# toybox-rs/Toybox

Hardware: AMD Instinct MI355X
Metric: env steps/sec (whole node), Breakout 64k-env batch (higher is better)
Workload: dtype f64

## Files before the change

toybox_amd/csrc/breakout.hip:

```cpp

#include "tbx_common.hpp"
#include "raster.hpp"
#include "agent_device.hpp"

#include <cstdlib>
#include <cstring>
#include <vector>

namespace {

constexpr int MAXB = TBX_BRK_MAX_BALLS;
constexpr int MAXK = TBX_BRK_MAX_BRICKS / 64;

struct BrkCustom {
    double x[TBX_BRK_MAX_BRICKS], y[TBX_BRK_MAX_BRICKS], w[TBX_BRK_MAX_BRICKS], h[TBX_BRK_MAX_BRICKS];
    int32_t points[TBX_BRK_MAX_BRICKS], depth[TBX_BRK_MAX_BRICKS], row[TBX_BRK_MAX_BRICKS], col[TBX_BRK_MAX_BRICKS];
    uint32_t color[TBX_BRK_MAX_BRICKS];
    uint8_t destructible[TBX_BRK_MAX_BRICKS];
};

struct BrkDev {
    int n;
    uint64_t* sim_rng;
    int32_t* prev_score;
// ... 1237 lines not shown
    const BrkRenderRec* __restrict__ recs, BrkPalette pal, uint8_t* __restrict__ out, int count, int split, BrkDev d, const BrkCfg* __restrict__ cp,
    ActionSource src, uint32_t flags, BrkRenderRec* __restrict__ recs_next, int step_blocks, unsigned long long* arrive, int release_block, int diag)
{
    if (!OVL) {
        if ((int)blockIdx.x < step_blocks) {
            const int env = (int)blockIdx.x * TBX_BLOCK + (int)threadIdx.x;
            if (env < d.n) brk_step_tpe_body<false, false>(d, *cp, src, flags, recs_next, nullptr, nullptr, env);
            return;
        }
        brk_render_body<C, false, false>(recs, nullptr, pal, out, 0, count, split | (1 << 16), nullptr, nullptr, (int)blockIdx.x - step_blocks);
        return;
    }
    if ((int)blockIdx.x < step_blocks) {
        const int env = (int)blockIdx.x * TBX_BLOCK + (int)threadIdx.x;
        if (OVL_DIAG(diag, 1)) {
            __builtin_amdgcn_fence(__ATOMIC_ACQUIRE, "agent");
            if (env < d.n) brk_step_tpe_body<false, false>(d, *cp, src, flags, recs_next, nullptr, nullptr, env);
            if (!OVL_DIAG(diag, 2)) __threadfence();
        } else {
            if (env < d.n) brk_step_tpe_body<false, true>(d, *cp, src, flags, recs_next, nullptr, nullptr, env);
            __builtin_amdgcn_s_waitcnt(0x0F70);
        }
        __syncthreads();
        if (threadIdx.x == 0) __hip_atomic_fetch_add(arrive, 1ull, __ATOMIC_RELAXED, __HIP_MEMORY_SCOPE_AGENT);
        return;
    }
    if ((int)blockIdx.x == release_block && threadIdx.x == 0) __hip_atomic_fetch_add(arrive + 1, 1ull, __ATOMIC_RELAXED, __HIP_MEMORY_SCOPE_AGENT);
    brk_render_body<C, false, false, true>(recs, nullptr, pal, out, 0, count, split | (1 << 16) | (OVL_DIAG(diag, 4) ? 1 << 17 : 0), nullptr, nullptr, (int)blockIdx.x - step_blocks);
}

template <int C, bool CUSTOM, bool ALT>
__global__ __launch_bounds__(TBX_BLOCK) void brk_render_kernel(const BrkRenderRec* __restrict__ recs, const BrkCustom* __restrict__ custom, BrkPalette pal,
                                                               uint8_t* __restrict__ out, int first_env, int count, int split,
                                                               const BrkRenderRec* __restrict__ recs_alt = nullptr, const uint8_t* __restrict__ pick_alt = nullptr)
{
    brk_render_body<C, CUSTOM, ALT>(recs, custom, pal, out, first_env, count, split, recs_alt, pick_alt, (int)blockIdx.x);
}

template <bool CUSTOM>
__device__ __forceinline__ bool brk_serve_paint(const BrkDev& d, const BrkRenderRec* recs, const BrkPalette& pal, int channels, uint8_t* frame, int lane, uint8_t* lds,
                                                int part, int split)
{
    const BrkRecLanes rec{brk_rec_load_lanes(&recs[0], lane)};
    switch (channels) {
    case 1: brk_paint_units<1, CUSTOM>(rec, d.custom, pal, BrkLaneTables<1>(pal, lane), frame, 0, lane, RowStager<1, TBX_BRK_W, BRK_UNIT_ROWS>{lds}, part, split); break;
    case 3: brk_paint_units<3, CUSTOM>(rec, d.custom, pal, BrkLaneTables<3>(pal, lane), frame, 0, lane, RowStager<3, TBX_BRK_W, BRK_UNIT_ROWS>{lds}, part, split); break;
    default: brk_paint_units<4, CUSTOM>(rec, d.custom, pal, BrkLaneTables<4>(pal, lane), frame, 0, lane, RowStager<4, TBX_BRK_W, BRK_UNIT_ROWS>{lds}, part, split); break;
    }
    return true;
}

template <bool CUSTOM>
__global__ __launch_bounds__(64 * TBX_SERVE_WAVES) void brk_serve_kernel(BrkDev d, BrkCfg c, BrkRenderRec* recs, BrkPalette pal, TbxServeCtl* ctl)
{
    __shared__ __attribute__((aligned(16))) uint8_t lds[TBX_SERVE_WAVES][RowStager<4, TBX_BRK_W, BRK_UNIT_ROWS>::UNIT_BYTES];
    const int lane = threadIdx.x & 63, wave = threadIdx.x >> 6;
    tbx_serve_loop(ctl, lane,
                   [&](const ActionSource& src, uint32_t flags) {
                       brk_step_body<CUSTOM>(d, c, src, flags, 0, lane);
                       __threadfence();
                       if (lane == 0) recs[0] = brk_record_of(d, 0);
                   },
                   [&](int channels, uint8_t* frame, int part, int split) { return brk_serve_paint<CUSTOM>(d, recs, pal, channels, frame, lane, lds[wave], part, split); },
                   d.reward, d.done, d.lives_out, d.score_out, d.err_flag);
}

__global__ __launch_bounds__(64 * TBX_SERVE_WAVES) void brk_serve_tpe_kernel(BrkDev d, const BrkCfg* __restrict__ cp, BrkRenderRec* recs, BrkPalette pal, TbxServeCtl* ctl)
{
    __shared__ __attribute__((aligned(16))) uint8_t lds[TBX_SERVE_WAVES][RowStager<4, TBX_BRK_W, BRK_UNIT_ROWS>::UNIT_BYTES];
    const int lane = threadIdx.x & 63, wave = threadIdx.x >> 6;
    tbx_serve_loop(ctl, lane, [&](const ActionSource& src, uint32_t flags) { if (lane == 0) brk_step_tpe_body<false>(d, *cp, src, flags, recs, nullptr, nullptr, 0); },
                   [&](int channels, uint8_t* frame, int part, int split) { return brk_serve_paint<false>(d, recs, pal, channels, frame, lane, lds[wave], part, split); },
                   d.reward, d.done, d.lives_out, d.score_out, d.err_flag);
}


struct BrkGrayPal {
    uint32_t bg, frame, paddle, ball;
    int32_t rows;
    uint32_t row[TBX_BRK_MAX_ROWS];
    uint64_t boundary[3];
};

struct BrkLineCache { int row; uint32_t dw; };

__device__ __forceinline__ uint32_t brk_gray_line(const BrkRenderRec& rec, const BrkGrayPal& pal, int y, int x0, uint32_t side_dw,
                                                  const uint32_t (&hud)[4], BrkLineCache& bc, bool has_overlay)
{
    uint32_t d;
    if (y < TBX_BRK_WALL_Y0) d = pal.bg * 0x01010101u;
    else if (y < TBX_BRK_WALL_Y0 + 12) d = pal.frame * 0x01010101u;
    else d = side_dw;
    const int by = y - 43;
    if (by >= 0 && by < 4 * pal.rows) {
        const int row = by >> 2;
        if (row != bc.row) {
            bc.row = row;
            uint32_t b = side_dw;
#pragma unroll
            for (int i = 0; i < 4; i++) {
                const int bxp = x0 + i - 12;
                if (bxp >= 0 && bxp < 216) {
                    const int j = (bxp / 12) * pal.rows + row;
                    const uint64_t w = sel4(j >> 6, rec.alive[0], rec.alive[1], rec.alive[2], rec.alive[3]);
                    if ((w >> (j & 63)) & 1ull) b = (b & ~(0xFFu << (8 * i))) | (pal.row[row] << (8 * i));
                }
            }
            bc.dw = b;
        }
        d = bc.dw;
    }
#pragma unroll
    for (int k = 0; k < 1 + MAXB; k++) {
        if (!has_overlay) break;
        const uint32_t rc = k == 0 ? rec.paddle : rec.ball[k - 1];
        const int ry0 = (int)((rc >> 16) & 255u), ry1 = (int)(rc >> 24);
        if (y >= ry0 && y < ry1) {
            const int rx0 = (int)(rc & 255u), rx1 = (int)((rc >> 8) & 255u);
            const uint32_t col = (k == 0 ? pal.paddle : pal.ball) * 0x01010101u;
            uint32_t m = 0;
#pragma unroll
            for (int i = 0; i < 4; i++)
                if (x0 + i >= rx0 && x0 + i < rx1) m |= 0xFFu << (8 * i);
            d = (d & ~m) | (col & m);
        }
    }
    if (y >= 2 && y < 12) {
        const int gr = ((y - 2) >> 1) * 3;
        uint32_t m = 0;
#pragma unroll
        for (int i = 0; i < 4; i++)
            if ((hud[i] >> gr) & 1u) m |= 0xFFu << (8 * i);
        d = (d & ~m) | ((pal.frame * 0x01010101u) & m);
    }
    return d;
}

template <int S>
__global__ __launch_bounds__(TBX_BLOCK) __attribute__((amdgpu_waves_per_eu(5))) void brk_agent_warp_kernel(const BrkRenderRec* __restrict__ recsLive, const BrkRenderRec* __restrict__ recsA,
                                                                   const BrkRenderRec* __restrict__ recsB, const BrkRenderRec* __restrict__ keepA,
                                                                   const BrkRenderRec* __restrict__ keepB, BrkGrayPal pal, AgentWarpArgs a, int n)
{
    constexpr int W = TBX_BRK_W, H = TBX_BRK_H;
    __shared__ __attribute__((aligned(16))) uint8_t lds_all[TBX_WAVES_PER_BLOCK][352];
    __shared__ __attribute__((aligned(16))) uint8_t vals_all[TBX_WAVES_PER_BLOCK][AGENT_MAX_OUT_PX];
    const int lane = threadIdx.x & 63;
    const int wave = threadIdx.x >> 6;
    const int env = wave_uniform(a.first + blockIdx.x * TBX_WAVES_PER_BLOCK + wave);
    if (env >= a.end) return;
    uint8_t* row = lds_all[wave];
    uint8_t* vals = vals_all[wave];
    const ObsSel sel = agent_obs_sel(a, env);
    if (sel.none) {
        for (int i = lane; i < a.oh * a.ow; i += 64) vals[i] = 0;
        observation_commit<S>(vals, a, env, lane, sel.zero);
        return;
    }
    const bool fresh = !sel.two;
    const BrkRenderRec* __restrict__ srcA = sel.keep ? keepA : recsA;
    const BrkRenderRec* __restrict__ srcB = sel.single == 0 ? recsLive : sel.single == 1 ? srcA : sel.keep ? keepB : recsB;
    const BrkRenderRec recA = srcA[env];
    const BrkRenderRec recB = srcB[env];
    const int x0 = lane * 4;
    const bool active = x0 < W;
    const uint32_t half = (uint32_t)(H * W) / 2u;
    const ColTaps c0 = load_col(a.tx, lane, a.ow), c1 = load_col(a.tx, lane + 64, a.ow);
    const bool on0 = lane < a.ow, on1 = lane + 64 < a.ow;
    if (lane < 8) reinterpret_cast<uint32_t*>(row)[80 + lane] = 0u;
    if (lane >= 60 && lane < 64) reinterpret_cast<uint32_t*>(row)[lane] = 0u;
    if (lane < 16) reinterpret_cast<uint32_t*>(row)[64 + lane] = 0u;

    uint32_t side_dw = 0;
#pragma unroll
    for (int i = 0; i < 4; i++) side_dw |= ((x0 + i < 12 || x0 + i >= 228) ? pal.frame : pal.bg) << (8 * i);
    uint32_t hudA[4], hudB[4];
    {
        const int hud_x0[7] = {36, 44, 52, 60, 68, 148, 196};
#pragma unroll
        for (int i = 0; i < 4; i++) {
            uint32_t sel = 7u << 2;
#pragma unroll
            for (int g = 0; g < 7; g++) {
                const int dx = x0 + i - hud_x0[g];
                if (dx >= 0 && dx < 6) sel = ((uint32_t)g << 2) | (uint32_t)(dx >> 1);
            }
            const uint32_t g = sel >> 2;
            const uint32_t ga = g < 7 ? tbx_digit_glyph((recA.hud >> (4 * g)) & 15u) : 0u;
            const uint32_t gb = g < 7 ? tbx_digit_glyph((recB.hud >> (4 * g)) & 15u) : 0u;
            hudA[i] = (ga >> (sel & 3u)) & 0x1249u;
            hudB[i] = (gb >> (sel & 3u)) & 0x1249u;
        }
    }

    BrkLineCache bcA{-1, 0}, bcB{-1, 0};
    uint64_t need[3] = {pal.boundary[0], pal.boundary[1], pal.boundary[2]};
    uint64_t ovA[3] = {0, 0, 0}, ovB[3] = {0, 0, 0}, diff_a[3] = {0, 0, 0};
    {
        brk_overlay_rows(recB, ovB);
        if (!fresh) brk_overlay_rows(recA, ovA);
        uint64_t ov[3];
#pragma unroll
        for (int w = 0; w < 3; w++) { ov[w] = ovA[w] | ovB[w]; need[w] |= ov[w]; diff_a[w] = fresh ? 0ull : ov[w]; }
        if (!fresh) {
            if (recA.alive[0] != recB.alive[0] || recA.alive[1] != recB.alive[1] || recA.alive[2] != recB.alive[2] ||
                recA.alive[3] != recB.alive[3] || recA.n_bricks != recB.n_bricks)
                brk_mark_rows(diff_a, 43, 43 + 4 * pal.rows);
            if (recA.hud != recB.hud) brk_mark_rows(diff_a, 2, 12);
        }
        need[2] |= (ov[2] << 1) | (ov[1] >> 63);
        need[1] |= (ov[1] << 1) | (ov[0] >> 63);
        need[0] |= (ov[0] << 1) | 1ull;
    }
    uint32_t h0 = 0, h1 = 0;
    uint32_t acc[2] = {0, 0};
    int oy = 0, top = H, pos = 0;
    auto run_to = [&](int end) {
        while (top <= end) {
            const uint32_t w = (uint32_t)(top - pos);
            const uint32_t s0 = acc[0] + __umul24(w, h0), s1 = acc[1] + __umul24(w, h1);
            if (on0) vals[oy * a.ow + lane] = (uint8_t)(((uint64_t)(s0 + half) * a.magic) >> 42);
            if (on1) vals[oy * a.ow + lane + 64] = (uint8_t)(((uint64_t)(s1 + half) * a.magic) >> 42);
            acc[0] = 0; acc[1] = 0;
            pos = top; top += H; oy += 1;
        }
        const uint32_t w = (uint32_t)(end - pos);
        acc[0] += __umul24(w, h0); acc[1] += __umul24(w, h1);
        pos = end;
    };
#pragma unroll 1
    for (int wi = 0; wi < 3; wi++) {
        uint64_t nw = sel4(wi, need[0], need[1], need[2], 0ull);
        const uint64_t oa = sel4(wi, ovA[0], ovA[1], ovA[2], 0ull), ob = sel4(wi, ovB[0], ovB[1], ovB[2], 0ull);
        const uint64_t da = sel4(wi, diff_a[0], diff_a[1], diff_a[2], 0ull);
        if (wi == 2) nw &= (1ull << (H - 128)) - 1ull;
#pragma unroll 1
        for (; nw; nw &= nw - 1ull) {
            const int b = (int)__builtin_ctzll(nw), sy = 64 * wi + b;
            run_to(sy * a.oh);
            const uint32_t dB = brk_gray_line(recB, pal, sy, x0, side_dw, hudB, bcB, (ob >> b) & 1ull);
            uint32_t v = dB;
            if ((da >> b) & 1ull) v = bytemax4(brk_gray_line(recA, pal, sy, x0, side_dw, hudA, bcA, (oa >> b) & 1ull), dB);
            if (active) reinterpret_cast<uint32_t*>(row)[lane] = v;
            __builtin_amdgcn_wave_barrier();
            h0 = on0 ? hsum(row, c0) : 0u;
            h1 = on1 ? hsum(row, c1) : 0u;
            __builtin_amdgcn_wave_barrier();
        }
    }
    run_to(H * a.oh);
    observation_commit<S>(vals, a, env, lane, sel.zero);
}


template <bool CUSTOM>
__global__ void brk_pack_kernel(BrkDev d, BrkCfg c, int env, tbx_breakout_state_t* out)
{
    env += blockIdx.x;
    out += blockIdx.x;
    const int lane = threadIdx.x & 63;
    BrkRegs s;
    brk_load(d, env, lane, s);
    if (lane == 0) {
        out->rand[0] = s.rng.s0; out->rand[1] = s.rng.s1;
        out->score = s.score; out->lives = s.lives; out->level = s.level;
        out->is_dead = (s.flags & 1) ? 1 : 0; out->reset = (s.flags & 2) ? 1 : 0;
        out->_pad0[0] = out->_pad0[1] = 0;
        out->paddle_x = s.px; out->paddle_y = s.py; out->paddle_vx = s.pvx; out->paddle_vy = s.pvy;
        out->paddle_width = s.pw; out->paddle_speed = s.pspeed; out->ball_radius = s.radius;
        out->n_balls = s.n_balls; out->n_bricks = s.n_bricks;
        for (int b = 0; b < MAXB; b++) {
            out->ball_x[b] = s.bx[b]; out->ball_y[b] = s.by[b]; out->ball_vx[b] = s.bvx[b]; out->ball_vy[b] = s.bvy[b];
        }
    }
    for (int k = 0; k < MAXK; k++) {
        const int j = lane + 64 * k;
        tbx_brick_t b;
        memset(&b, 0, sizeof b);
        if (j < s.n_bricks) {
            if (CUSTOM) {
                const BrkCustom& t = d.custom[env];
                b.x = t.x[j]; b.y = t.y[j]; b.w = t.w[j]; b.h = t.h[j];
                b.points = t.points[j]; b.depth = t.depth[j]; b.row = t.row[j]; b.col = t.col[j];
                b.color = unpack_color(t.color[j]); b.destructible = t.destructible[j];
            } else {
                int row, col;
                brk_canon(j, c.n_rows, row, col, b.x, b.y);
                b.w = TBX_BRK_BRICK_W; b.h = TBX_BRK_BRICK_H;
                b.points = c.row_scores[row]; b.depth = c.n_rows - 1 - row; b.row = row; b.col = col;
                b.color = unpack_color(c.row_colors[row]); b.destructible = 1;
            }
            b.alive = (s.mybits >> k) & 1u;
        }
        out->bricks[j] = b;
    }
}

template <bool CUSTOM>
__global__ void brk_unpack_kernel(BrkDev d, int env, const tbx_breakout_state_t* in)
{
    env += blockIdx.x;
    in += blockIdx.x;
    const int lane = threadIdx.x & 63;
    BrkRegs s;
    s.rng.s0 = in->rand[0]; s.rng.s1 = in->rand[1];
    s.score = in->score; s.lives = in->lives; s.level = in->level;
    s.flags = (in->is_dead ? 1 : 0) | (in->reset ? 2 : 0);
    s.px = in->paddle_x; s.py = in->paddle_y; s.pvx = in->paddle_vx; s.pvy = in->paddle_vy;
    s.pw = in->paddle_width; s.pspeed = in->paddle_speed; s.radius = in->ball_radius;
    s.n_balls = in->n_balls; s.n_bricks = in->n_bricks;
    for (int b = 0; b < MAXB; b++) {
        const bool v = b < s.n_balls;
        s.bx[b] = v ? in->ball_x[b] : 0.0; s.by[b] = v ? in->ball_y[b] : 0.0;
        s.bvx[b] = v ? in->ball_vx[b] : 0.0; s.bvy[b] = v ? in->ball_vy[b] : 0.0;
    }
    uint32_t bits = 0;
    for (int k = 0; k < MAXK; k++) {
        const int j = lane + 64 * k;
        const tbx_brick_t& b = in->bricks[j];
        if (j < s.n_bricks && b.alive) bits |= 1u << k;
        if (CUSTOM) {
            BrkCustom& t = d.custom[env];
            const bool v = j < s.n_bricks;
            t.x[j] = v ? b.x : 0.0; t.y[j] = v ? b.y : 0.0; t.w[j] = v ? b.w : 0.0; t.h[j] = v ? b.h : 0.0;
            t.points[j] = v ? b.points : 0; t.depth[j] = v ? b.depth : 0; t.row[j] = v ? b.row : 0; t.col[j] = v ? b.col : 0;
            t.color[j] = v ? pack_color(b.color) : 0u; t.destructible[j] = v ? (b.destructible ? 1 : 0) : 0;
        }
    }
    s.mybits = bits;
    brk_store(d, env, lane, s);
}

__global__ __launch_bounds__(TBX_BLOCK) void brk_fill_custom_kernel(BrkDev d, BrkCfg c)
{
// ... 90 lines not shown
        o[0] = c;
        break;
    }
    case TBX_QUERY_BRK_NUM_BRICKS: o[0] = nb; break;
    case TBX_QUERY_BRK_COLUMN: case TBX_QUERY_BRK_ROW: {
        const int key = a.geti(env, 0);
        int m = 0;
        for (int j = 0; j < nb && m < width; j++) {
            int row, col;
            brk_brick_rc<CUSTOM>(d, env, j, rows, row, col);
            if ((query == TBX_QUERY_BRK_COLUMN ? col : row) == key) o[m++] = alive(j);
        }
        for (; m < width; m++) o[m] = -1.0;
        break;
    }
    case TBX_QUERY_BRK_IS_CHANNEL: case TBX_QUERY_BRK_CHANNEL_COUNT: case TBX_QUERY_BRK_FIND_CHANNEL: {
        const int ncols = query == TBX_QUERY_BRK_IS_CHANNEL ? 0 : (rows > 0 ? nb / rows : 0);
        const int want = a.geti(env, 0);
        int count = 0, first = -1, is = 0;
        const int c0 = query == TBX_QUERY_BRK_IS_CHANNEL ? want : 0, c1 = query == TBX_QUERY_BRK_IS_CHANNEL ? want + 1 : ncols;
        for (int cc = c0; cc < c1; cc++) {
            int bricks = 0, live = 0;
            for (int j = 0; j < nb; j++) {
                int row, col;
                brk_brick_rc<CUSTOM>(d, env, j, rows, row, col);
                if (col == cc) { bricks++; live += alive(j); }
            }
            if (bricks > 0 && live == 0) { count++; if (first < 0) first = cc; is = 1; }
        }
        o[0] = query == TBX_QUERY_BRK_IS_CHANNEL ? is : query == TBX_QUERY_BRK_CHANNEL_COUNT ? count : first;
        break;
    }
    case TBX_QUERY_BRK_FIND_BRICK: {
        const int want = a.geti(env, 0);
        int first = -1;
        for (int j = 0; j < nb && first < 0; j++)
            if (((a.getu(env, 1 + (j >> 5)) >> (j & 31)) & 1u) && (want < 0 || alive(j) == (want != 0))) first = j;
        o[0] = first;
        break;
    }
    case TBX_QUERY_BRK_PADDLE:
        for (int i = 0; i < 4; i++) o[i] = d.paddle[(size_t)i * N + env];
        break;
    case TBX_QUERY_BRK_BALLS: {
        const int n = d.n_balls[env];
        o[0] = n;
        for (int f = 0; f < 4; f++)
            for (int b = 0; b < MAXB; b++) o[1 + f * MAXB + b] = b < n ? d.balls[(size_t)(f * MAXB + b) * N + env] : -1.0;
        break;
    }
    default: break;
    }
}

__global__ void brk_scalars_kernel(BrkDev d, int32_t* score, int32_t* lives, int32_t* level)
{
    const int i = blockIdx.x * blockDim.x + threadIdx.x;
    if (i >= d.n) return;
    if (score) score[i] = d.score[i];
    if (lives) lives[i] = d.lives[i];
    if (level) level[i] = d.level[i];
}


struct BrkSlots {
    BrkRenderRec *recsA, *recsB;
    BrkRenderRec *keepA, *keepB;
    template <class F>
    constexpr void arrays(F&& f)
    {
        f(recsA, tbx_rows(sizeof(BrkRenderRec))); f(recsB, tbx_rows(sizeof(BrkRenderRec)));
        f(keepA, tbx_rows(sizeof(BrkRenderRec))); f(keepB, tbx_rows(sizeof(BrkRenderRec)));
    }
};
static_assert(sizeof(BrkSlots) == sizeof(void*) * tbx_array_count<BrkSlots>(), "BrkSlots: the arrays of arrays()");

struct BreakoutOps : GameOps {
    BrkDev d{};
    BrkCfg c{};
    tbx_breakout_config_t cfg{};
    bool custom = false;
    TbxRecordSet<BrkRenderRec> recs;
    BrkCfg* cfg_dev = nullptr;

    static void default_config(tbx_breakout_config_t* k);

    int height() const override { return TBX_BRK_H; }
    int width() const override { return TBX_BRK_W; }
    size_t state_size() const override { return sizeof(tbx_breakout_state_t); }
    size_t config_size() const override { return sizeof(tbx_breakout_config_t); }

    int load_cfg(tbx_engine* e, const tbx_breakout_config_t& k)
    {
        if (k.n_rows < 1 || k.n_rows > TBX_BRK_MAX_ROWS) return e->fail(TBX_E_UNSUPPORTED, "breakout: n_rows must be 1..14");
        if (k.n_starts < 1 || k.n_starts > TBX_BRK_MAX_STARTS) return e->fail(TBX_E_UNSUPPORTED, "breakout: 1..8 ball_start_positions");
        if (k.paddle_discrete_segments < 1 || k.paddle_discrete_segments > TBX_BRK_MAX_SEGMENTS)
            return e->fail(TBX_E_UNSUPPORTED, "breakout: paddle_discrete_segments must be 1..16 (continuous bounce needs device trig)");
        cfg = k;
        c.start_lives = k.start_lives; c.n_rows = k.n_rows; c.ball_speed_row_depth = k.ball_speed_row_depth;
        c.n_starts = k.n_starts; c.segments = k.paddle_discrete_segments;
        for (int i = 0; i < TBX_BRK_MAX_ROWS; i++) { c.row_scores[i] = k.row_scores[i]; c.row_colors[i] = pack_color(k.row_colors[i]); }
        c.speed_slow = k.ball_speed_slow; c.speed_fast = k.ball_speed_fast;
        for (int i = 0; i < TBX_BRK_MAX_STARTS; i++) {
            c.start_x[i] = k.start_x[i]; c.start_y[i] = k.start_y[i];
            c.start_dx[i] = k.start_dir_x[i]; c.start_dy[i] = k.start_dir_y[i];
        }
        for (int i = 0; i < TBX_BRK_MAX_SEGMENTS; i++) { c.pad_dx[i] = k.paddle_dir_x[i]; c.pad_dy[i] = k.paddle_dir_y[i]; }
        c.bg = pack_color(k.bg_color); c.frame = pack_color(k.frame_color);
        c.paddle = pack_color(k.paddle_color); c.ball = pack_color(k.ball_color);
        if (!cfg_dev) TBX_HIP(hipMalloc((void**)&cfg_dev, sizeof(BrkCfg)));
        TBX_HIP(hipMemcpy(cfg_dev, &c, sizeof(BrkCfg), hipMemcpyHostToDevice));
        return TBX_OK;
    }

    int init(tbx_engine* e, const void* cfg_pod, size_t cfg_size) override
    {
        tbx_breakout_config_t k;
        if (cfg_pod) {
            if (cfg_size != sizeof k) return e->fail(TBX_E_INVALID, "breakout: config size mismatch");
            memcpy(&k, cfg_pod, sizeof k);
        } else {
            return e->fail(TBX_E_INVALID, "breakout: a config record is required");
        }
        int rc = load_cfg(e, k);
        if (rc) return rc;
        options_changed(e);
        tbx_bind_engine(d, e);
        TBX_HIP(tbx_alloc_arrays(d, (size_t)e->n));
        TBX_HIP(recs.alloc((size_t)e->n, 3));
        return TBX_OK;
    }

    void destroy(tbx_engine*) override
    {
        tbx_free_arrays(d);
        tbx_free_arrays(slots);
        recs.release();
        hipFree(cfg_dev);
    }

    int get_config(tbx_engine*, void* pod) override { memcpy(pod, &cfg, sizeof cfg); return TBX_OK; }
    int set_config(tbx_engine* e, const void* pod) override
    {
        tbx_breakout_config_t k;
        memcpy(&k, pod, sizeof k);
        return load_cfg(e, k);
    }

    int new_game(tbx_engine* e, const uint8_t* mask_dev, hipStream_t s) override
    {
        tbx_dispatch<0, 1>(custom, [&](auto cu) { hipLaunchKernelGGL(brk_new_game_kernel<decltype(cu)::value != 0>, grid_for(e->n), dim3(TBX_BLOCK), 0, s, d, c, mask_dev); });
        TBX_HIP(hipGetLastError());
        recs.valid = false;
        return TBX_OK;
    }

    int step(tbx_engine* e, const ActionSource& src, uint32_t flags, hipStream_t s) override
    {
        if (!custom && src.single_env < 0 && use_tpe) {
            if (src.acc_reward || src.buf_valid || src.exec_flag || src.frames > 1) {
                if (flags & TBX_STEP_AUTO_RESET) return e->fail(TBX_E_INVALID, "an agent step cannot auto-reset");
                hipLaunchKernelGGL(brk_step_tpe_kernel<true>, dim3((e->n + 127) / 128), dim3(128), 0, s, d, cfg_dev, src, flags, recs.cur, slots.recsA, slots.recsB);
            } else
                TBX_LAUNCH_STEP(e, s, (brk_step_tpe_kernel<false>), dim3((e->n + 127) / 128), dim3(128), d, cfg_dev, src, flags, recs.cur, slots.recsA, slots.recsB);
            TBX_HIP(hipGetLastError());
            recs.valid = true;
// ... 131 lines not shown
            tbx_dispatch<0, 1>(custom, [&](auto cu) {
                tbx_dispatch<0, 1>(pick_alt != nullptr, [&](auto al) {
                    if (C >= 3) BRK_LAUNCH(brk_render_kernel_w5);
                    else BRK_LAUNCH(brk_render_kernel);
                });
            });
#undef BRK_LAUNCH
        };
        constexpr int HEAD_ENVS = 1024;
        if (two_parts) { launch_part(0, HEAD_ENVS); launch_part(HEAD_ENVS, count - HEAD_ENVS); }
        else launch_part(0, count);
    }

    int render(tbx_engine* e, uint8_t* out_dev, int channels, int first_env, int n_envs, hipStream_t s) override
    {
        if (!tbx_dispatch<1, 3, 4>(channels, [&](auto ch) { launch_render<decltype(ch)::value>(out_dev, first_env, n_envs, s); }))
            return e->fail(TBX_E_INVALID, "channels must be 1, 3 or 4");
        TBX_HIP(hipGetLastError());
        return TBX_OK;
    }

    BrkSlots slots{};

    bool agent_fused() const override { return !custom; }
    bool multi_frame_step() const override { return !custom && use_tpe; }
    bool agent_reset_supported() const override { return !custom; }

    int agent_prepare(tbx_engine* e) override
    {
        if (!slots.recsA) TBX_HIP(tbx_alloc_arrays(slots, (size_t)e->n));
        TBX_HIP(tbx_zero_arrays(slots, (size_t)e->n));
        return TBX_OK;
    }

    int agent_snapshot(tbx_engine* e, int slot, const uint8_t* exec_flag, uint8_t* buf_valid, hipStream_t s) override
    {
        hipLaunchKernelGGL(brk_render_prep_kernel, dim3((e->n + 255) / 256), dim3(256), 0, s, d, slot ? slots.recsB : slots.recsA, 0, e->n, exec_flag,
                           buf_valid, slot ? 2 : 1);
        TBX_HIP(hipGetLastError());
        return TBX_OK;
    }

    int render_from(tbx_engine* e, int source, const uint8_t* pick_live, uint8_t* out_dev, int channels, hipStream_t s) override
    {
        const BrkRenderRec* src_recs = source == 1 ? slots.recsA : source == 2 ? slots.recsB : nullptr;
        const BrkRenderRec* alt = (src_recs && pick_live) ? recs.cur : nullptr;
        if (!tbx_dispatch<1, 3, 4>(channels, [&](auto ch) { launch_render<decltype(ch)::value>(out_dev, 0, e->n, s, src_recs, alt, alt ? pick_live : nullptr); }))
            return e->fail(TBX_E_INVALID, "channels must be 1, 3 or 4");
        TBX_HIP(hipGetLastError());
        return TBX_OK;
    }

    int agent_reset_envs(tbx_engine* e, const AgentResetArgs& r, hipStream_t s) override
    {
        if (custom) return e->fail(TBX_E_UNSUPPORTED, "breakout: episodic-life / fire-reset / no-op-reset need the canonical brick wall");
        hipLaunchKernelGGL(brk_agent_reset_kernel, dim3((e->n + 127) / 128), dim3(128), 0, s, d, cfg_dev, r, recs.cur, slots.recsA, slots.recsB, slots.keepA, slots.keepB);
        TBX_HIP(hipGetLastError());
        return TBX_OK;
    }

    static uint32_t host_gray(uint32_t rgba)
    {
        const uint32_t r = rgba & 255u, g = (rgba >> 8) & 255u, b = (rgba >> 16) & 255u;
        return (77u * r + 150u * g + 29u * b + 128u) >> 8;
    }

    int agent_warp(tbx_engine* e, const AgentWarpArgs& a, hipStream_t s) override
    {
        BrkGrayPal pal;
        pal.bg = host_gray(c.bg); pal.frame = host_gray(c.frame); pal.paddle = host_gray(c.paddle); pal.ball = host_gray(c.ball);
        pal.rows = c.n_rows;
        for (int i = 0; i < TBX_BRK_MAX_ROWS; i++) pal.row[i] = host_gray(c.row_colors[i]);
        pal.boundary[0] = pal.boundary[1] = pal.boundary[2] = 0;
        auto mark = [&](int y) { if (y >= 0 && y < TBX_BRK_H) pal.boundary[y >> 6] |= 1ull << (y & 63); };
        mark(0);
        for (int y = 2; y <= 12; y += 2) mark(y);
        mark(TBX_BRK_WALL_Y0); mark(TBX_BRK_WALL_Y0 + 12);
        for (int r = 0; r <= c.n_rows; r++) mark(43 + 4 * r);
        if (!recs.valid) {
            hipLaunchKernelGGL(brk_render_prep_kernel, dim3((e->n + 255) / 256), dim3(256), 0, s, d, recs.cur, 0, e->n);
            TBX_HIP(hipGetLastError());
            recs.valid = true;
        }
        const dim3 grid = grid_for(a.end - a.first), block(TBX_BLOCK);
        tbx_dispatch<0, 1, 2, 3, 4>(tbx_stack_arm(a.obs, a.stack), [&](auto depth) {
            hipLaunchKernelGGL(brk_agent_warp_kernel<decltype(depth)::value>, grid, block, 0, s, recs.cur, slots.recsA, slots.recsB, slots.keepA, slots.keepB, pal, a, e->n);
        });
        TBX_HIP(hipGetLastError());
        return TBX_OK;
    }

    int pack_state(tbx_engine* e, int env, int count, hipStream_t s) override
    {
        auto* out = (tbx_breakout_state_t*)e->staging.p;
        tbx_dispatch<0, 1>(custom, [&](auto cu) { hipLaunchKernelGGL(brk_pack_kernel<decltype(cu)::value != 0>, dim3(count), dim3(64), 0, s, d, c, env, out); });
        TBX_HIP(hipGetLastError());
        return TBX_OK;
    }

    bool is_canonical(const tbx_breakout_state_t& st) const
    {
        if (st.n_bricks != TBX_BRK_COLS * cfg.n_rows) return false;
        for (int j = 0; j < st.n_bricks; j++) {
            const tbx_brick_t& b = st.bricks[j];
            const int col = j / cfg.n_rows, row = j % cfg.n_rows;
            if (b.x != TBX_BRK_LEFT + TBX_BRK_BRICK_W * col || b.y != TBX_BRK_BRICK_Y0 + TBX_BRK_BRICK_H * row ||
                b.w != TBX_BRK_BRICK_W || b.h != TBX_BRK_BRICK_H || b.points != cfg.row_scores[row] ||
                b.depth != cfg.n_rows - 1 - row || b.row != row || b.col != col || !b.destructible ||
                pack_color(b.color) != pack_color(cfg.row_colors[row]))
                return false;
        }
        return true;
    }

    int enable_custom(tbx_engine* e, hipStream_t s)
    {
        if (custom) return TBX_OK;
        TBX_HIP(tbx_alloc_arrays(d, (size_t)e->n, true));
        hipLaunchKernelGGL(brk_fill_custom_kernel, grid_for(e->n), dim3(TBX_BLOCK), 0, s, d, c);
        TBX_HIP(hipGetLastError());
        custom = true;
        return TBX_OK;
    }

    int unpack_state(tbx_engine* e, int env, int count, const void* pod_host, hipStream_t s) override
    {
        const auto* sts = (const tbx_breakout_state_t*)pod_host;
        bool all_canonical = true;
        for (int i = 0; i < count; i++) {
            const auto& st = sts[i];
            if (st.n_balls < 0 || st.n_balls > TBX_BRK_MAX_BALLS)
                return e->fail(TBX_E_UNSUPPORTED, "breakout: the device engine holds at most 4 balls per env");
            if (st.n_bricks < 0 || st.n_bricks > TBX_BRK_MAX_BRICKS)
                return e->fail(TBX_E_UNSUPPORTED, "breakout: the device engine holds at most 256 bricks per env");
            if (!custom && all_canonical && !is_canonical(st)) all_canonical = false;
        }
        if (!custom && !all_canonical) {
            int rc = enable_custom(e, s);
            if (rc) return rc;
        }
        TBX_HIP(hipMemcpyAsync(e->staging.p, pod_host, sizeof(tbx_breakout_state_t) * (size_t)count, hipMemcpyHostToDevice, s));
        auto* in = (const tbx_breakout_state_t*)e->staging.p;
        tbx_dispatch<0, 1>(custom, [&](auto cu) { hipLaunchKernelGGL(brk_unpack_kernel<decltype(cu)::value != 0>, dim3(count), dim3(64), 0, s, d, env, in); });
        TBX_HIP(hipGetLastError());
        recs.valid = false;
        return TBX_OK;
    }

    int edit(tbx_engine* e, int op, const TbxEditArgs& a, const uint8_t* mask_dev, hipStream_t s) override
    {
        switch (op) {
        case TBX_EDIT_SET_LIVES: case TBX_EDIT_SET_SCORE: case TBX_EDIT_SET_LEVEL: case TBX_EDIT_BRK_COLUMN_ALIVE: case TBX_EDIT_BRK_ROW_ALIVE:
        case TBX_EDIT_BRK_ALL_ALIVE: case TBX_EDIT_BRK_BRICK_ALIVE: case TBX_EDIT_BRK_PADDLE: case TBX_EDIT_BRK_BALL: break;
        default: return e->fail(TBX_E_INVALID, "breakout: unknown edit");
        }
        const dim3 grid((e->n + 255) / 256), block(256);
        tbx_dispatch<0, 1>(custom, [&](auto cu) { hipLaunchKernelGGL(brk_edit_kernel<decltype(cu)::value != 0>, grid, block, 0, s, d, c.n_rows, op, a, mask_dev); });
        TBX_HIP(hipGetLastError());
        recs.valid = false;
        return TBX_OK;
    }

    int lookahead(tbx_engine* e, const TbxEditArgs& a, bool all, double* out_dev, hipStream_t s) override
    {
        const int cands = all ? tbx_legal_count(TBX_GAME_BREAKOUT) : 1;
        tbx_lookahead_launches(e->n, cands, [&](long long p0, int count) {
            if (!custom && use_tpe) hipLaunchKernelGGL(brk_lookahead_tpe_kernel, dim3((count + 127) / 128), dim3(128), 0, s, d, cfg_dev, a, cands, p0, count, out_dev);
// ... 63 lines not shown
```

Baseline: 54.56 million.

## Make Breakout observation kernel persistent with lane-distributed record decode

Converts the agent observation kernel to a grid-stride persistent loop capped at five blocks per CU, so per-lane setup (column taps, lane constants) is done once per wave instead of once per env. Each lane loads one dword of the render record and uses bpermute/broadcast to derive brick bits, HUD glyphs and overlay rows, which replaces per-pixel branchy loops with precomputed masks. Per-lane predicates are removed by zeroing taps and padding the vals buffer. The trade-off is more LDS per block and reliance on helper functions (brk_rec_load_lanes, bcast) whose layout must match the record.

Result: no change. 54.63 million, median of 2 (+0.1%).

```diff
diff --git a/toybox_amd/csrc/breakout.hip b/toybox_amd/csrc/breakout.hip
--- a/toybox_amd/csrc/breakout.hip
+++ b/toybox_amd/csrc/breakout.hip
@@ -1343,59 +1343,112 @@
     uint64_t boundary[3];
 };
 
-struct BrkLineCache { int row; uint32_t dw; };
-
-__device__ __forceinline__ uint32_t brk_gray_line(const BrkRenderRec& rec, const BrkGrayPal& pal, int y, int x0, uint32_t side_dw,
-                                                  const uint32_t (&hud)[4], BrkLineCache& bc, bool has_overlay)
-{
-    uint32_t d;
-    if (y < TBX_BRK_WALL_Y0) d = pal.bg * 0x01010101u;
-    else if (y < TBX_BRK_WALL_Y0 + 12) d = pal.frame * 0x01010101u;
-    else d = side_dw;
+struct BrkObsLane {
+    uint32_t side_dw;
+    uint32_t keep;
+    uint32_t row_dw;
+    int brick_addr;
+    uint32_t brick_sh, brick_mask;
+    uint32_t hud_shift, hud_c0, hud_mask;
+};
+
+__device__ __forceinline__ BrkObsLane brk_obs_lane(const BrkGrayPal& pal, int lane)
+{
+    BrkObsLane k;
+    const int x0 = lane * 4;
+    k.side_dw = ((x0 < 12 || x0 >= 228) ? pal.frame : pal.bg) * 0x01010101u;
+    k.keep = x0 < TBX_BRK_W ? ~0u : 0u;
+    k.row_dw = 0u;
+#pragma unroll
+    for (int r = 0; r < TBX_BRK_MAX_ROWS; r++)
+        if (lane == r) k.row_dw = pal.row[r] * 0x01010101u;
+    const bool wall = lane >= 3 && lane < 57;
+    const int j0 = wall ? ((lane - 3) / 3) * pal.rows : 0;
+    k.brick_addr = (j0 >> 5) * 4;
+    k.brick_sh = (uint32_t)(j0 & 31);
+    k.brick_mask = wall ? (1u << pal.rows) - 1u : 0u;
+    k.hud_shift = 0u; k.hud_c0 = 0u; k.hud_mask = 0u;
+    const int hud_x0[7] = {36, 44, 52, 60, 68, 148, 196};
+#pragma unroll
+    for (int g = 0; g < 7; g++) {
+        if (x0 == hud_x0[g]) { k.hud_shift = 4u * g; k.hud_c0 = 0u; k.hud_mask = 0x36DBu; }
+        if (x0 == hud_x0[g] + 4) { k.hud_shift = 4u * g; k.hud_c0 = 2u; k.hud_mask = 0x1249u; }
+    }
+    return k;
+}
+static_assert(TBX_BRK_MAX_ROWS * TBX_BRK_COLS <= 252 && TBX_BRK_MAX_ROWS <= 16, "a lane's brick column: rows bits that end inside the four alive words");
+
+__device__ __forceinline__ uint32_t brk_xmask4(uint32_t rc, int x0)
+{
+    const int rx0 = (int)(rc & 255u), rx1 = (int)((rc >> 8) & 255u);
+    const int lo = min(max(rx0 - x0, 0), 4), hi = min(max(rx1 - x0, 0), 4);
+    const uint32_t below_hi = (uint32_t)((0xFFFFFFFFull << (8 * hi)) >> 32), below_lo = (uint32_t)((0xFFFFFFFFull << (8 * lo)) >> 32);
+    return below_hi & ~below_lo;
+}
+
+struct BrkObsRec {
+    uint32_t bricks;
+    uint32_t glyph;
+    uint32_t xm[1 + MAXB];
+    uint32_t y0[1 + MAXB], h[1 + MAXB];
+    uint32_t hud;
+};
+
+__device__ __forceinline__ BrkObsRec brk_obs_rec(uint32_t rv, const BrkObsLane& k, int lane)
+{
+    BrkObsRec r;
+    const uint32_t lo = (uint32_t)__builtin_amdgcn_ds_bpermute(k.brick_addr, (int)rv), hi = (uint32_t)__builtin_amdgcn_ds_bpermute(k.brick_addr + 4, (int)rv);
+    r.bricks = __builtin_amdgcn_alignbit(hi, lo, k.brick_sh) & k.brick_mask;
+    r.hud = bcast(rv, 13);
+    r.glyph = (tbx_digit_glyph((r.hud >> k.hud_shift) & 15u) >> k.hud_c0) & k.hud_mask;
+#pragma unroll
+    for (int i = 0; i < 1 + MAXB; i++) {
+        const uint32_t rc = bcast(rv, 8 + i);
+        const uint32_t ry0 = (rc >> 16) & 255u, ry1 = rc >> 24;
+        r.y0[i] = ry0;
+        r.h[i] = ((rc & 255u) < ((rc >> 8) & 255u) && ry1 > ry0) ? ry1 - ry0 : 0u;
+        r.xm[i] = brk_xmask4(rc, lane * 4);
+    }
+    return r;
+}
+
+__device__ __forceinline__ void brk_obs_overlay_rows(const BrkObsRec& r, int lane, uint64_t (&m)[3])
+{
+#pragma unroll
+    for (int w = 0; w < 3; w++) {
+        bool in = false;
+#pragma unroll
+        for (int i = 0; i < 1 + MAXB; i++) in |= (uint32_t)(lane + 64 * w) - r.y0[i] < r.h[i];
+        m[w] = __builtin_amdgcn_ballot_w64(in);
+    }
+}
+
+__device__ __forceinline__ uint32_t brk_gray_line(const BrkObsRec& rec, const BrkGrayPal& pal, const BrkObsLane& k, int y, bool has_overlay)
+{
+    const uint32_t frame_dw = pal.frame * 0x01010101u;
+    uint32_t d = y < TBX_BRK_WALL_Y0 ? pal.bg * 0x01010101u : y < TBX_BRK_WALL_Y0 + 12 ? frame_dw : k.side_dw;
     const int by = y - 43;
     if (by >= 0 && by < 4 * pal.rows) {
         const int row = by >> 2;
-        if (row != bc.row) {
-            bc.row = row;
-            uint32_t b = side_dw;
-#pragma unroll
-            for (int i = 0; i < 4; i++) {
-                const int bxp = x0 + i - 12;
-                if (bxp >= 0 && bxp < 216) {
-                    const int j = (bxp / 12) * pal.rows + row;
-                    const uint64_t w = sel4(j >> 6, rec.alive[0], rec.alive[1], rec.alive[2], rec.alive[3]);
-                    if ((w >> (j & 63)) & 1ull) b = (b & ~(0xFFu << (8 * i))) | (pal.row[row] << (8 * i));
-                }
-            }
-            bc.dw = b;
-        }
-        d = bc.dw;
-    }
-#pragma unroll
-    for (int k = 0; k < 1 + MAXB; k++) {
-        if (!has_overlay) break;
-        const uint32_t rc = k == 0 ? rec.paddle : rec.ball[k - 1];
-        const int ry0 = (int)((rc >> 16) & 255u), ry1 = (int)(rc >> 24);
-        if (y >= ry0 && y < ry1) {
-            const int rx0 = (int)(rc & 255u), rx1 = (int)((rc >> 8) & 255u);
-            const uint32_t col = (k == 0 ? pal.paddle : pal.ball) * 0x01010101u;
-            uint32_t m = 0;
-#pragma unroll
-            for (int i = 0; i < 4; i++)
-                if (x0 + i >= rx0 && x0 + i < rx1) m |= 0xFFu << (8 * i);
-            d = (d & ~m) | (col & m);
+        const uint32_t m = 0u - ((rec.bricks >> row) & 1u);
+        d = (k.side_dw & ~m) | (bcast(k.row_dw, row) & m);
+    }
+    if (has_overlay) {
+#pragma unroll
+        for (int i = 0; i < 1 + MAXB; i++) {
+            const uint32_t m = ((uint32_t)y - rec.y0[i] < rec.h[i]) ? rec.xm[i] : 0u;
+            d = (d & ~m) | (((i == 0 ? pal.paddle : pal.ball) * 0x01010101u) & m);
         }
     }
     if (y >= 2 && y < 12) {
-        const int gr = ((y - 2) >> 1) * 3;
-        uint32_t m = 0;
-#pragma unroll
-        for (int i = 0; i < 4; i++)
-            if ((hud[i] >> gr) & 1u) m |= 0xFFu << (8 * i);
-        d = (d & ~m) | ((pal.frame * 0x01010101u) & m);
+        const uint32_t t = rec.glyph >> (((y - 2) >> 1) * 3);
+        const uint32_t m = ((t & 1u) ? 0x0000FFFFu : 0u) | ((t & 2u) ? 0xFFFF0000u : 0u);
+        d = (d & ~m) | (frame_dw & m);
     }
     return d;
 }
+
+constexpr int BRK_OBS_VALS_PAD = 128;
 
 template <int S>
 __global__ __launch_bounds__(TBX_BLOCK) __attribute__((amdgpu_waves_per_eu(5))) void brk_agent_warp_kernel(const BrkRenderRec* __restrict__ recsLive, const BrkRenderRec* __restrict__ recsA,
@@ -1404,112 +1457,92 @@
 {
     constexpr int W = TBX_BRK_W, H = TBX_BRK_H;
     __shared__ __attribute__((aligned(16))) uint8_t lds_all[TBX_WAVES_PER_BLOCK][352];
-    __shared__ __attribute__((aligned(16))) uint8_t vals_all[TBX_WAVES_PER_BLOCK][AGENT_MAX_OUT_PX];
+    __shared__ __attribute__((aligned(16))) uint8_t vals_all[TBX_WAVES_PER_BLOCK][AGENT_MAX_OUT_PX + BRK_OBS_VALS_PAD];
     const int lane = threadIdx.x & 63;
     const int wave = threadIdx.x >> 6;
-    const int env = wave_uniform(a.first + blockIdx.x * TBX_WAVES_PER_BLOCK + wave);
+    const int n_waves = (int)gridDim.x * TBX_WAVES_PER_BLOCK;
+    int env = wave_uniform(a.first + blockIdx.x * TBX_WAVES_PER_BLOCK + wave);
     if (env >= a.end) return;
     uint8_t* row = lds_all[wave];
     uint8_t* vals = vals_all[wave];
-    const ObsSel sel = agent_obs_sel(a, env);
-    if (sel.none) {
-        for (int i = lane; i < a.oh * a.ow; i += 64) vals[i] = 0;
+    const uint32_t half = (uint32_t)(H * W) / 2u;
+    const BrkObsLane k = brk_obs_lane(pal, lane);
+    ColTaps c0 = load_col(a.tx, lane, a.ow), c1 = load_col(a.tx, lane + 64, a.ow);
+    if (lane >= a.ow) { c0.wlo = 0u; c0.whi = 0u; }
+    if (lane + 64 >= a.ow) { c1.wlo = 0u; c1.whi = 0u; }
+    if (lane < 24) reinterpret_cast<uint32_t*>(row)[64 + lane] = 0u;
+
+#pragma unroll 1
+    for (; env < a.end; env += n_waves) {
+        const ObsSel sel = agent_obs_sel(a, env);
+        if (sel.none) {
+            for (int i = lane; i < a.oh * a.ow; i += 64) vals[i] = 0;
+            observation_commit<S>(vals, a, env, lane, sel.zero);
+            continue;
+        }
+        const bool fresh = !sel.two;
+        const BrkRenderRec* __restrict__ srcA = sel.keep ? keepA : recsA;
+        const BrkRenderRec* __restrict__ srcB = sel.single == 0 ? recsLive : sel.single == 1 ? srcA : sel.keep ? keepB : recsB;
+        const uint32_t rvB = brk_rec_load_lanes(&srcB[env], lane);
+        const uint32_t rvA = fresh ? rvB : brk_rec_load_lanes(&srcA[env], lane);
+        const BrkObsRec recB = brk_obs_rec(rvB, k, lane);
+        const BrkObsRec recA = fresh ? recB : brk_obs_rec(rvA, k, lane);
+
+        uint64_t need[3] = {pal.boundary[0], pal.boundary[1], pal.boundary[2]};
+        uint64_t ovA[3] = {0, 0, 0}, ovB[3] = {0, 0, 0}, diff_a[3] = {0, 0, 0};
+        {
+            brk_obs_overlay_rows(recB, lane, ovB);
+            if (!fresh) brk_obs_overlay_rows(recA, lane, ovA);
+            uint64_t ov[3];
+#pragma unroll
+            for (int w = 0; w < 3; w++) { ov[w] = ovA[w] | ovB[w]; need[w] |= ov[w]; diff_a[w] = fresh ? 0ull : ov[w]; }
+            if (!fresh) {
+                if (__builtin_amdgcn_ballot_w64(recA.bricks != recB.bricks) != 0ull) brk_mark_rows(diff_a, 43, 43 + 4 * pal.rows);
+                if (recA.hud != recB.hud) brk_mark_rows(diff_a, 2, 12);
+            }
+            need[2] |= (ov[2] << 1) | (ov[1] >> 63);
+            need[1] |= (ov[1] << 1) | (ov[0] >> 63);
+            need[0] |= (ov[0] << 1) | 1ull;
+        }
+        uint32_t h0 = 0, h1 = 0;
+        uint32_t acc[2] = {0, 0};
+        int oy = 0, top = H, pos = 0;
+        auto run_to = [&](int end) {
+#pragma clang loop vectorize(disable) interleave(disable)
+            while (top <= end) {
+                const uint32_t w = (uint32_t)(top - pos);
+                const uint32_t s0 = acc[0] + __umul24(w, h0), s1 = acc[1] + __umul24(w, h1);
+                vals[oy * a.ow + lane] = (uint8_t)(((uint64_t)(s0 + half) * a.magic) >> 42);
+                vals[oy * a.ow + lane + 64] = (uint8_t)(((uint64_t)(s1 + half) * a.magic) >> 42);
+                acc[0] = 0; acc[1] = 0;
+                pos = top; top += H; oy += 1;
+            }
+            const uint32_t w = (uint32_t)(end - pos);
+            acc[0] += __umul24(w, h0); acc[1] += __umul24(w, h1);
+            pos = end;
+        };
+#pragma unroll 1
+        for (int wi = 0; wi < 3; wi++) {
+            uint64_t nw = sel4(wi, need[0], need[1], need[2], 0ull);
+            const uint64_t oa = sel4(wi, ovA[0], ovA[1], ovA[2], 0ull), ob = sel4(wi, ovB[0], ovB[1], ovB[2], 0ull);
+            const uint64_t da = sel4(wi, diff_a[0], diff_a[1], diff_a[2], 0ull);
+            if (wi == 2) nw &= (1ull << (H - 128)) - 1ull;
+#pragma unroll 1
+            for (; nw; nw &= nw - 1ull) {
+                const int b = (int)__builtin_ctzll(nw), sy = 64 * wi + b;
+                run_to(sy * a.oh);
+                uint32_t v = brk_gray_line(recB, pal, k, sy, (ob >> b) & 1ull);
+                if ((da >> b) & 1ull) v = bytemax4(brk_gray_line(recA, pal, k, sy, (oa >> b) & 1ull), v);
+                reinterpret_cast<uint32_t*>(row)[lane] = v & k.keep;
+                __builtin_amdgcn_wave_barrier();
+                h0 = hsum(row, c0);
+                h1 = hsum(row, c1);
+                __builtin_amdgcn_wave_barrier();
+            }
+        }
+        run_to(H * a.oh);
         observation_commit<S>(vals, a, env, lane, sel.zero);
-        return;
-    }
-    const bool fresh = !sel.two;
-    const BrkRenderRec* __restrict__ srcA = sel.keep ? keepA : recsA;
-    const BrkRenderRec* __restrict__ srcB = sel.single == 0 ? recsLive : sel.single == 1 ? srcA : sel.keep ? keepB : recsB;
-    const BrkRenderRec recA = srcA[env];
-    const BrkRenderRec recB = srcB[env];
-    const int x0 = lane * 4;
-    const bool active = x0 < W;
-    const uint32_t half = (uint32_t)(H * W) / 2u;
-    const ColTaps c0 = load_col(a.tx, lane, a.ow), c1 = load_col(a.tx, lane + 64, a.ow);
-    const bool on0 = lane < a.ow, on1 = lane + 64 < a.ow;
-    if (lane < 8) reinterpret_cast<uint32_t*>(row)[80 + lane] = 0u;
-    if (lane >= 60 && lane < 64) reinterpret_cast<uint32_t*>(row)[lane] = 0u;
-    if (lane < 16) reinterpret_cast<uint32_t*>(row)[64 + lane] = 0u;
-
-    uint32_t side_dw = 0;
-#pragma unroll
-    for (int i = 0; i < 4; i++) side_dw |= ((x0 + i < 12 || x0 + i >= 228) ? pal.frame : pal.bg) << (8 * i);
-    uint32_t hudA[4], hudB[4];
-    {
-        const int hud_x0[7] = {36, 44, 52, 60, 68, 148, 196};
-#pragma unroll
-        for (int i = 0; i < 4; i++) {
-            uint32_t sel = 7u << 2;
-#pragma unroll
-            for (int g = 0; g < 7; g++) {
-                const int dx = x0 + i - hud_x0[g];
-                if (dx >= 0 && dx < 6) sel = ((uint32_t)g << 2) | (uint32_t)(dx >> 1);
-            }
-            const uint32_t g = sel >> 2;
-            const uint32_t ga = g < 7 ? tbx_digit_glyph((recA.hud >> (4 * g)) & 15u) : 0u;
-            const uint32_t gb = g < 7 ? tbx_digit_glyph((recB.hud >> (4 * g)) & 15u) : 0u;
-            hudA[i] = (ga >> (sel & 3u)) & 0x1249u;
-            hudB[i] = (gb >> (sel & 3u)) & 0x1249u;
-        }
-    }
-
-    BrkLineCache bcA{-1, 0}, bcB{-1, 0};
-    uint64_t need[3] = {pal.boundary[0], pal.boundary[1], pal.boundary[2]};
-    uint64_t ovA[3] = {0, 0, 0}, ovB[3] = {0, 0, 0}, diff_a[3] = {0, 0, 0};
-    {
-        brk_overlay_rows(recB, ovB);
-        if (!fresh) brk_overlay_rows(recA, ovA);
-        uint64_t ov[3];
-#pragma unroll
-        for (int w = 0; w < 3; w++) { ov[w] = ovA[w] | ovB[w]; need[w] |= ov[w]; diff_a[w] = fresh ? 0ull : ov[w]; }
-        if (!fresh) {
-            if (recA.alive[0] != recB.alive[0] || recA.alive[1] != recB.alive[1] || recA.alive[2] != recB.alive[2] ||
-                recA.alive[3] != recB.alive[3] || recA.n_bricks != recB.n_bricks)
-                brk_mark_rows(diff_a, 43, 43 + 4 * pal.rows);
-            if (recA.hud != recB.hud) brk_mark_rows(diff_a, 2, 12);
-        }
-        need[2] |= (ov[2] << 1) | (ov[1] >> 63);
-        need[1] |= (ov[1] << 1) | (ov[0] >> 63);
-        need[0] |= (ov[0] << 1) | 1ull;
-    }
-    uint32_t h0 = 0, h1 = 0;
-    uint32_t acc[2] = {0, 0};
-    int oy = 0, top = H, pos = 0;
-    auto run_to = [&](int end) {
-        while (top <= end) {
-            const uint32_t w = (uint32_t)(top - pos);
-            const uint32_t s0 = acc[0] + __umul24(w, h0), s1 = acc[1] + __umul24(w, h1);
-            if (on0) vals[oy * a.ow + lane] = (uint8_t)(((uint64_t)(s0 + half) * a.magic) >> 42);
-            if (on1) vals[oy * a.ow + lane + 64] = (uint8_t)(((uint64_t)(s1 + half) * a.magic) >> 42);
-            acc[0] = 0; acc[1] = 0;
-            pos = top; top += H; oy += 1;
-        }
-        const uint32_t w = (uint32_t)(end - pos);
-        acc[0] += __umul24(w, h0); acc[1] += __umul24(w, h1);
-        pos = end;
-    };
-#pragma unroll 1
-    for (int wi = 0; wi < 3; wi++) {
-        uint64_t nw = sel4(wi, need[0], need[1], need[2], 0ull);
-        const uint64_t oa = sel4(wi, ovA[0], ovA[1], ovA[2], 0ull), ob = sel4(wi, ovB[0], ovB[1], ovB[2], 0ull);
-        const uint64_t da = sel4(wi, diff_a[0], diff_a[1], diff_a[2], 0ull);
-        if (wi == 2) nw &= (1ull << (H - 128)) - 1ull;
-#pragma unroll 1
-        for (; nw; nw &= nw - 1ull) {
-            const int b = (int)__builtin_ctzll(nw), sy = 64 * wi + b;
-            run_to(sy * a.oh);
-            const uint32_t dB = brk_gray_line(recB, pal, sy, x0, side_dw, hudB, bcB, (ob >> b) & 1ull);
-            uint32_t v = dB;
-            if ((da >> b) & 1ull) v = bytemax4(brk_gray_line(recA, pal, sy, x0, side_dw, hudA, bcA, (oa >> b) & 1ull), dB);
-            if (active) reinterpret_cast<uint32_t*>(row)[lane] = v;
-            __builtin_amdgcn_wave_barrier();
-            h0 = on0 ? hsum(row, c0) : 0u;
-            h1 = on1 ? hsum(row, c1) : 0u;
-            __builtin_amdgcn_wave_barrier();
-        }
-    }
-    run_to(H * a.oh);
-    observation_commit<S>(vals, a, env, lane, sel.zero);
+    }
 }
 
 
@@ -1766,6 +1799,7 @@
     bool custom = false;
     TbxRecordSet<BrkRenderRec> recs;
     BrkCfg* cfg_dev = nullptr;
+    unsigned obs_blocks = 0;
 
     static void default_config(tbx_breakout_config_t* k);
 
@@ -2063,7 +2097,12 @@
             TBX_HIP(hipGetLastError());
             recs.valid = true;
         }
-        const dim3 grid = grid_for(a.end - a.first), block(TBX_BLOCK);
+        if (!obs_blocks) {
+            int cus = 0;
+            TBX_HIP(hipDeviceGetAttribute(&cus, hipDeviceAttributeMultiprocessorCount, e->device));
+            obs_blocks = 5u * (unsigned)std::max(cus, 1);
+        }
+        const dim3 grid(std::min(grid_for(a.end - a.first).x, obs_blocks)), block(TBX_BLOCK);
         tbx_dispatch<0, 1, 2, 3, 4>(tbx_stack_arm(a.obs, a.stack), [&](auto depth) {
             hipLaunchKernelGGL(brk_agent_warp_kernel<decltype(depth)::value>, grid, block, 0, s, recs.cur, slots.recsA, slots.recsB, slots.keepA, slots.keepB, pal, a, e->n);
         });
```
